# jzi040941/PercepNet

Hardware: AMD Instinct MI355X
Metric: real-time 48 kHz streams (10 ms frames), whole job (higher is better)
Workload: dtype f32; 1 GPU; configs[2]: 65536 concurrent 48 kHz streams per MI355X, fp32 network as MFMA GEMM; streams_per_gpu=65536, frame_samples=480, nn_mode=mfma_f32, weights=torch.manual_seed(1234) default-init PercepNet in nnet_data.h layout, parallelism=streams sharded over 1 GPU(s), one process per GPU, no data-path collective, io=int16 PCM in, int16 PCM + g|r rows out, resident in HBM, distributed=none (plain process)

## Files before the change

### percepnet_amd/build.py

```python
import os
import subprocess
import sys

HERE = os.path.dirname(os.path.abspath(__file__))
CSRC = os.path.join(HERE, "csrc")
LIBDIR = os.path.join(HERE, "lib")
LIB = os.path.join(LIBDIR, "libpercepnet_hip.so")
RUN = os.path.join(LIBDIR, "percepnet_run")
EXPORT_MAP = os.path.join(CSRC, "libpercepnet_hip.map")
SOURCES = ["pn_tables.cpp", "pn_model.cpp", "pn_pack.cpp", "pn_dsp_fe.hip", "pn_dsp_fe_g2.hip", "pn_dsp_fe_split_s.hip", "pn_dsp_fe_split_p.hip", "pn_dsp.hip", "pn_outstage.hip", "pn_nn.hip", "pn_nn_small.hip", "pn_nn_x3.hip", "pn_nn_d.hip", "pn_nn_n48.hip", "pn_targets.hip", "pn_state.hip", "pn_active.hip", "pn_stream_state.hip", "pn_context.cpp", "pn_selftest.cpp", "pn_host_pipe.cpp", "pn_stream_state.cpp", "pn_network.cpp",
           "pn_featgen.cpp", "pn_rate.hip", "pn_rate.cpp", "rnnoise_compat.cpp"]
FLAGS = ["--offload-arch=gfx950", "-O3", "-std=c++17", "-ffp-contract=off", "-fPIC", "-fvisibility=hidden",
         "-Wall", "-Wno-unused-function", "-Wno-unused-variable", "-Wno-unused-value", "-Wno-unused-result"]


EXTRA_FLAGS = {"pn_nn_x3.hip": ["-fno-slp-vectorize", "-mllvm", "-pragma-unroll-threshold=1000000"],
               "pn_nn_d.hip": ["-fno-slp-vectorize"]}


def _hipcc():
    for c in (os.environ.get("HIPCC"), "/opt/rocm/bin/hipcc", "hipcc"):
        if c and (os.path.isabs(c) and os.path.exists(c) or not os.path.isabs(c)):
            return c
    raise RuntimeError("hipcc not found")


EXPECTED_HIP = "7.2"

RESOURCE_LIMITS = {"pn_fe_spec_in_kernel": (0, 0), "pn_fe_spec_out_kernel": (0, 40), "pn_fe_pitch_kernel": (0, 48),
                   "pn_backend_kernel": (0, 16),
                   "pn_gru_x3_kernel": (0, 0), "pn_dense_x3_kernel": (0, 0),
                   "pn_gru_d_kernel": (0, 0)}
RESOURCE_SOURCES = ("pn_dsp_fe_split_s.hip", "pn_dsp_fe_split_p.hip", "pn_dsp.hip", "pn_nn_x3.hip", "pn_nn_d.hip")


def parse_resource_remarks(text):
    import re
    out, cur = {}, None
    for line in text.splitlines():
        m = re.search(r"remark: .*Function Name: (\S+)", line)
        if m:
            name = m.group(1)
            mm = re.match(r"_Z\d+(pn_[a-z0-9_]+)", name)
            cur = out.setdefault(name, {"kernel": mm.group(1) if mm else name})
            continue
        m = re.search(r"remark: .*?\s+(VGPRs|AGPRs|ScratchSize \[bytes/lane\]|Occupancy \[waves/SIMD\]|LDS Size \[bytes/block\]|VGPRs Spill|SGPRs Spill): (\d+)", line)
        if m and cur is not None:
            cur[m.group(1).split(" [")[0]] = int(m.group(2))
    return out


def check_resources(remarks):
    bad = []
    for name, r in remarks.items():
        for prefix, (max_agpr, max_scratch) in RESOURCE_LIMITS.items():
            if r["kernel"].startswith(prefix):
                if r.get("AGPRs", 0) > max_agpr or r.get("ScratchSize", 0) > max_scratch:
                    bad.append(f"{r['kernel']}: {r.get('VGPRs')} VGPRs, {r.get('AGPRs')} AGPRs, {r.get('ScratchSize')} B/lane scratch "
                               f"(limits: {max_agpr} AGPRs, {max_scratch} B) [{name}]")
    return bad


LLVM_BIN = "/opt/rocm/lib/llvm/bin"
GATED_OBJECTS = ("pn_dsp_fe_split_p",)


def disassemble_device_code(obj_path):
    import shutil
    import tempfile
    objdump = os.path.join(LLVM_BIN, "llvm-objdump")
    if not os.path.exists(objdump):
        objdump = shutil.which("llvm-objdump")
    if not objdump:
        raise RuntimeError("llvm-objdump not found: the disassembly gate cannot run")
    with tempfile.TemporaryDirectory() as d:
        local = os.path.join(d, os.path.basename(obj_path))
        shutil.copy(obj_path, local)
        subprocess.run([objdump, "--offloading", local], cwd=d, capture_output=True, text=True, check=True)
        cos = [f for f in os.listdir(d) if "amdgcn" in f]
        if not cos:
            raise RuntimeError(f"no device code object in {obj_path}")
        return subprocess.run([objdump, "-d", os.path.join(d, cos[0])], capture_output=True, text=True, check=True).stdout


def _vregs(op):
    import re
    m = re.fullmatch(r"v(\d+)", op)
    if m:
        return {int(m.group(1))}
    m = re.fullmatch(r"v\[(\d+):(\d+)\]", op)
    return set(range(int(m.group(1)), int(m.group(2)) + 1)) if m else set()


def check_dpp_and_waitcnt(disasm):
    import re
    bad = []
    func, ins = None, []
    funcs = {}
    for line in disasm.splitlines():
        m = re.match(r"^[0-9a-f]+ <([^>]+)>:", line)
        if m:
            func = m.group(1); ins = funcs.setdefault(func, [])
            continue
        t = line.split("//")[0].strip()
        if func is None or not t or t.startswith("."):
            continue
        parts = t.split(None, 1)
        ops = [o.strip() for o in re.split(r",\s*(?![^\[]*\])", parts[1])] if len(parts) > 1 else []
        ins.append((parts[0], ops, t))
    for func, ins in funcs.items():
        for i, (mn, ops, text) in enumerate(ins):
            if "_dpp" not in mn or len(ops) < 2:
# ... 134 lines not shown
```

### percepnet_amd/csrc/pn_context.cpp

```cpp
#include "pn_context.h"
#include <stdio.h>
#include <float.h>
#include <math.h>

extern "C" int pn_device_count(void) { int n = 0; return hipGetDeviceCount(&n) == hipSuccess ? n : 0; }


static thread_local bool g_last_alloc_oom = false;
bool &last_alloc_oom() { return g_last_alloc_oom; }
int dev_alloc_into(std::vector<void *> &allocs, size_t &total, hipStream_t stream, void **p, size_t bytes, bool zero) {
  static const bool guard = getenv("PERCEPNET_GUARD") != NULL;
  const size_t pad = guard ? (1u << 20) : 0, body = (bytes + 255) & ~(size_t)255;
  {
    const hipError_t e = hipMalloc(p, guard ? body + pad : bytes);
    if (e != hipSuccess) {
      g_last_alloc_oom = (e == hipErrorOutOfMemory);
      (void)hipGetLastError();
      pn_set_error("hipMalloc(%zu bytes) failed: %s", bytes, hipGetErrorString(e));
      return -1;
    }
  }
  allocs.push_back(*p);
  total += bytes;
  if (zero) PN_HIP_CHECK(hipMemsetAsync(*p, 0, bytes, stream));
// ... 160 lines not shown
  }
  return 0;
}
extern "C" int pn_ctx_n_streams(const pn_ctx *c) { return c ? c->B : -1; }
extern "C" int64_t pn_ctx_frames_done(const pn_ctx *c) { return c ? c->t : -1; }
extern "C" size_t pn_ctx_device_bytes(const pn_ctx *c) { return c ? c->bytes + ((c->weights && !c->weights_were_cached) ? c->weight_bytes : 0) : 0; }
extern "C" size_t pn_ctx_weight_bytes(const pn_ctx *c) { return (c && c->weights) ? c->weight_bytes : 0; }
extern "C" int pn_ctx_describe(const pn_ctx *c, char *buf, size_t n) {
  if (!c || !buf || !n) return -1;
  const int f = pn_plan_describe(c->plan, c->nn_mode, buf, n);
  if (f < 0 || (size_t)f >= n) return -1;
  const int k = c->plan.chains;
  const int w = f + snprintf(buf + f, n - f, " weights=%s nn_chains=%d%s%s", c->weights_were_cached ? "shared" : "own", k, k > 1 ? ":" : "", k > 1 ? c->chain_kind + 1 : "");
  if (w < 0 || (size_t)w >= n) return -1;
  if (c->x3_sat) {
    DeviceGuard _dg(c->device);
    hipStreamSynchronize(c->stream);
    const int w2 = snprintf(buf + w, n - w, " x3_saturated=%lld", pn_x3_sat_read());
    return (w2 < 0 || (size_t)(w + w2) >= n) ? -1 : w + w2;
  }
  return w;
}
extern "C" int pn_ctx_synchronize(pn_ctx *c) { if (!c) return -1; PN_ON_DEVICE(c); PN_HIP_CHECK(hipStreamSynchronize(c->stream)); return 0; }


static int flush_events(pn_ctx *c) {
  PN_HIP_CHECK(hipStreamSynchronize(c->stream));
  for (int k = 1; k < 4; k++) if (c->chain_stream[k]) PN_HIP_CHECK(hipStreamSynchronize(c->chain_stream[k]));
  for (auto &e : c->events) {
    float ms = 0;
    if (hipEventElapsedTime(&ms, e.a, e.b) == hipSuccess) { c->fam_ms[e.fam] += ms; c->fam_n[e.fam]++; }
    c->event_pool.push_back(e.a); c->event_pool.push_back(e.b);
  }
  c->events.clear();
  return 0;
}

extern "C" int pn_ctx_set_profiling(pn_ctx *c, int enable) {
  if (!c) return -1;
  if (enable && c->event_pool.size() < 2048) {
    PN_ON_DEVICE(c);
    while (c->event_pool.size() < 2048) { hipEvent_t e; PN_HIP_CHECK(hipEventCreate(&e)); c->event_pool.push_back(e); }
  }
  c->profiling = enable != 0;
  return 0;
}
extern "C" int pn_kernel_count(void) { return KF_COUNT; }
extern "C" const char *pn_kernel_name(int i) { return (i >= 0 && i < KF_COUNT) ? pn_kFamilyName[i] : NULL; }
extern "C" int pn_ctx_kernel_time(pn_ctx *c, const char *name, double *total_ms, int64_t *launches) {
  if (!c || !name) return -1;
  if (flush_events(c)) return -1;
  for (int i = 0; i < KF_COUNT; i++)
    if (!strcmp(name, pn_kFamilyName[i])) { if (total_ms) *total_ms = c->fam_ms[i]; if (launches) *launches = c->fam_n[i]; return 0; }
  pn_set_error("unknown kernel family '%s'", name);
  return -1;
}
extern "C" int pn_ctx_reset_profile(pn_ctx *c) {
  if (!c) return -1;
  if (flush_events(c)) return -1;
  memset(c->fam_ms, 0, sizeof(c->fam_ms)); memset(c->fam_n, 0, sizeof(c->fam_n));
  return 0;
}

void pn_launch_fe(hipStream_t st, const PnTables *T, int n_streams, int fe, int k, const PnDspSide &s, const PnDspSlots &sl, const PnDspIn &in, int grid_cap) {
  static PnFeLaunch *const launch[][3] = {{pn_launch_frontend}, {pn_launch_frontend_g2}, {pn_launch_fe_spec_in, pn_launch_fe_pitch, pn_launch_fe_spec_out}};
  static_assert(sizeof(launch) / sizeof(launch[0]) == sizeof(pn_kFe) / sizeof(pn_kFe[0]) && sizeof(launch[0]) / sizeof(launch[0][0]) == sizeof(pn_kFe[0].fam) / sizeof(int),
                "one row of launchers per front-end family of pn_kFe");
  launch[fe][k](st, T, n_streams, s, sl, in, grid_cap);
}

int process_dev(pn_ctx *c, const void *d_in, void *d_out, float *d_gr, int is_i16) {
  if (!c || !d_in || !d_out) { pn_set_error("NULL argument"); return -1; }
  PN_ON_DEVICE(c);
  const PnDspSide &s = c->side;
  const PnDspSlots k = pn_dsp_slots(c->t);
  const PnDspIn in = {d_in, is_i16, PN_FRAME, 1.f / 32768.f};
  float *const gr = c->st[PN_ST_GR].p;
  for (int i = 0; i < pn_kFe[c->plan.fe].n; i++) {
    Scope sc(c, pn_kFe[c->plan.fe].fam[i]);
    pn_launch_fe(c->stream, c->tables, c->B, c->plan.fe, i, s, k, in, c->dsp_grid_cap);
  }
  if (launch_rnn(c)) return -1;
  const bool stage = c->report_on || (c->saturate && is_i16), staged_cast = stage && is_i16;
  { Scope sc(c, KF_BACKEND);
    pn_launch_backend(c->stream, c->tables, c->B, pn_dsp_spec(s, k.slot_r), s.Ps, gr, c->postfilter ? pn_dsp_bands(s, k.slot_r) : nullptr, s.silence,
                      c->st[PN_ST_SYNTH].p, staged_cast ? (void *)c->stage_o : d_out, staged_cast ? 0 : is_i16, c->dsp_grid_cap,
                      c->n_limited > 0 ? c->lam_mu : nullptr); }
  if (stage) {
    Scope sc(c, KF_BACKEND);
    pn_launch_outstage(c->stream, c->B, staged_cast ? c->stage_o : (const float *)d_out, s, (k.frame_t + 6) % PN_HIST_FRAMES, gr,
                       is_i16 ? (int16_t *)d_out : nullptr, c->saturate, c->report_on ? c->report : nullptr);
  }
  if (d_gr) PN_HIP_CHECK(hipMemcpyAsync(d_gr, gr, (size_t)c->B * 68 * 4, hipMemcpyDeviceToDevice, c->stream));
  PN_HIP_CHECK(hipGetLastError());
  c->t++; c->tn++;
  if (c->events.size() >= 4096 && flush_events(c)) return -1;
  return 0;
}

extern "C" int pn_ctx_debug_inject_launch_failure(pn_ctx *c, int enable) {
  if (!c) { pn_set_error("NULL argument"); return -1; }
  c->inject_bad_launch = enable != 0;
  return 0;
}

extern "C" int pn_ctx_set_postfilter(pn_ctx *c, int enable) {
  if (!c) { pn_set_error("NULL argument"); return -1; }
  c->postfilter = enable != 0;
  return 0;
}

static int stage_buffers(pn_ctx *c, bool report) {
  if (!c->stage_o && dev_alloc(c, (void **)&c->stage_o, (size_t)c->B * PN_FRAME * sizeof(float), false)) return -1;
  if (report && !c->report && dev_alloc(c, (void **)&c->report, (size_t)c->B * PN_REPORT_WORDS * 4, true)) return -1;
  return 0;
}
extern "C" int pn_ctx_set_report(pn_ctx *c, int enable) {
  if (!c) { pn_set_error("NULL argument"); return -1; }
  if (enable) { PN_ON_DEVICE(c); if (stage_buffers(c, true)) return -1; }
  else c->next_report = NULL;
  c->report_on = enable != 0;
  return 0;
}
extern "C" int pn_ctx_set_output_saturate(pn_ctx *c, int enable) {
  if (!c) { pn_set_error("NULL argument"); return -1; }
  if (enable) { PN_ON_DEVICE(c); if (stage_buffers(c, false)) return -1; }
  c->saturate = enable != 0;
  return 0;
}
static int report_copy(pn_ctx *c, void *dst, hipMemcpyKind kind) {
  if (!c || !dst) { pn_set_error("NULL argument"); return -1; }
  if (!c->report_on) { pn_set_error("the frame report is off (pn_ctx_set_report)"); return -1; }
  PN_ON_DEVICE(c);
  PN_HIP_CHECK(hipMemcpyAsync(dst, c->report, (size_t)c->B * PN_REPORT_WORDS * 4, kind, c->stream));
  if (kind == hipMemcpyDeviceToHost) PN_HIP_CHECK(hipStreamSynchronize(c->stream));
  return 0;
}
extern "C" int pn_ctx_read_report(pn_ctx *c, void *h_report) { return report_copy(c, h_report, hipMemcpyDeviceToHost); }
extern "C" int pn_ctx_read_report_dev(pn_ctx *c, void *d_report) { return report_copy(c, d_report, hipMemcpyDeviceToDevice); }

extern "C" float pn_atten_limit_factor(float db) {
  if (!(db >= 0.f)) return NAN;
  const float lam = (float)pow(10.0, -(double)db / 20.0);
  return lam < FLT_MIN ? 0.f : lam;
}
extern "C" int pn_ctx_set_atten_limit(pn_ctx *c, const int32_t *ids, int n, const float *db) {
  if (!c || (n > 0 && !db)) { pn_set_error("bad argument"); return -1; }
  if (pn_ids_check(c->B, ids, n, true)) return -1;
  if (n == 0) return 0;
  for (int i = 0; i < n; i++) {
    if (!(db[i] >= 0.f)) { pn_set_error("attenuation limit %g dB for stream %d: must be >= 0 (+inf = off)", (double)db[i], ids[i]); return -1; }
  }
  PN_ON_DEVICE(c);
  if (!c->lam_mu && dev_alloc(c, (void **)&c->lam_mu, (size_t)c->B * sizeof(float2), true)) return -1;
  std::vector<float2> lm(n);
  for (int i = 0; i < n; i++) { const float lam = pn_atten_limit_factor(db[i]); lm[i] = make_float2(lam, 1.0f - lam); }
  const int *d = stage_ids(c, ids, n, lm.data(), 2 * n);
  if (!d) return -1;
  pn_launch_scatter_pairs(c->stream, c->lam_mu, d, reinterpret_cast<const float2 *>(d + stage_payload_offset(n)), n);
  PN_HIP_CHECK(hipGetLastError());
  for (int i = 0; i < n; i++) {
    c->n_limited += (lm[i].x != 0.f) - (pn_atten_limit_factor(c->atten_db[ids[i]]) != 0.f);
    c->atten_db[ids[i]] = db[i];
  }
  return 0;
}
extern "C" int pn_ctx_get_atten_limit(const pn_ctx *c, float *h_db) {
  if (!c || !h_db) { pn_set_error("bad argument"); return -1; }
  memcpy(h_db, c->atten_db.data(), (size_t)c->B * sizeof(float));
  return 0;
}

extern "C" int pn_process_f32(pn_ctx *c, const float *d_in, float *d_out, float *d_gr) { return process_dev(c, d_in, d_out, d_gr, 0); }
extern "C" int pn_process_i16(pn_ctx *c, const int16_t *d_in, int16_t *d_out, float *d_gr) { return process_dev(c, d_in, d_out, d_gr, 1); }
extern "C" int pn_process_i16_multi(pn_ctx *c, const int16_t *d_in, int16_t *d_out, float *d_gr, int n_frames) {
  if (!c) return -1;
// ... 106 lines not shown
```

### percepnet_amd/csrc/pn_dsp.hip

```cpp
#include "pn_fft960.h"
#include "pn_launch.h"
#include "pn_pcm.h"

#define LANES 64
#ifndef PN_DSP_WPB
#define PN_DSP_WPB 8
#endif
#ifndef PN_DSP_WAVES_PER_SIMD
#define PN_DSP_WAVES_PER_SIMD 4
#endif
#define WPB PN_DSP_WPB
#define DSP_THREADS (LANES * WPB)

#define PN_WAVE_SYNC_GLOBAL() do { __builtin_amdgcn_fence(__ATOMIC_SEQ_CST, "workgroup"); __builtin_amdgcn_wave_barrier(); } while (0)

struct alignas(16) PnDspWaveLds {
  float2 fft[FS_NF];
  float e[4][PN_NB + 2];
};
struct PnDspShared {
  float win[PN_FRAME];
  float frac[PN_SPEC_BINS];
  uint8_t band[PN_SPEC_BINS];
  PnDspWaveLds w[WPB];
};

template <typename P, typename... R> __device__ __forceinline__ P pn_first_arg(P p, R...) { return p; }

template <typename TOut, bool PF, typename... LamMu>
__global__ __launch_bounds__(DSP_THREADS, PN_DSP_WAVES_PER_SIMD) void pn_backend_kernel(
    const PnTables *__restrict__ T, int n_streams,
    const float2 *__restrict__ Xspec, const float2 *__restrict__ Pspec,
    const float *__restrict__ gr,
    const float *__restrict__ ex,
    const int *__restrict__ silence,
    float *__restrict__ synth_mem,
    TOut *__restrict__ out,
    const LamMu *__restrict__... lam_mu) {
  constexpr bool AL = sizeof...(LamMu) != 0;
  __shared__ PnDspShared SH;
  const int tid = threadIdx.x, lane = tid & (LANES - 1), wave = __builtin_amdgcn_readfirstlane(tid >> 6);
  for (int i = tid; i < PN_FRAME; i += DSP_THREADS) SH.win[i] = T->half_window[i];
  for (int i = tid; i < PN_SPEC_BINS; i += DSP_THREADS) { SH.frac[i] = T->bin_frac[i]; SH.band[i] = T->bin_band[i]; }
  __syncthreads();
  PnDspWaveLds &W = SH.w[wave];
  FsLane Z;
  fs_lane_init(Z, T, lane);
  const float scale = 1.f / PN_NFFT;
  const int lc = lane < 60 ? lane : 59;
  for (int s = blockIdx.x * WPB + wave; s < n_streams; s += gridDim.x * WPB) {
    const bool sil = silence[s] != 0;
    float lam = 0.f, mu = 0.f;
    if constexpr (AL) { const float2 lm = pn_first_arg(lam_mu...)[s]; lam = lm.x; mu = lm.y; }
    const bool mix = AL && lam != 0.f;
    if (lane < PN_NB) {
      const float g = gr[(size_t)s * 68 + lane], r = gr[(size_t)s * 68 + PN_NB + lane];
      W.e[0][lane] = g; W.e[1][lane] = r; W.e[2][lane] = 1 - r;
      if (PF) W.e[3][lane] = ex[(size_t)s * 36 + lane];
    }
    PN_WAVE_SYNC();
    if (PF) {
      float gw = 0.f;
      float *gws = reinterpret_cast<float *>(W.fft);
      if (lane < PN_NB) { const float g = W.e[0][lane]; gw = g * sinf((float)(M_PI / 2 * (double)g)); gws[lane] = gw; }
      PN_WAVE_SYNC();
      float E0 = 0.f, E1 = 0.f;
#pragma unroll 2
      for (int i = 0; i < PN_NB; i++) {
        const float e = W.e[3][i];
        E0 += W.e[0][i] * e;
        E1 += gws[i] * e;
      }
      const float E_div = E0 / (E1 + 1e-6f);
      const float G = sqrtf(((1 + 0.02f) * E_div) / (1 + 0.02f * (E_div * E_div)));
      PN_WAVE_SYNC();
      if (lane < PN_NB) W.e[0][lane] = G * gw;
      PN_WAVE_SYNC();
    }
    {
      const float4 *X4 = reinterpret_cast<const float4 *>(Xspec + (size_t)s * PN_SPEC_BINS);
      const float4 *P4 = reinterpret_cast<const float4 *>(Pspec + (size_t)s * PN_SPEC_BINS);
      float4 xq[4], pq[4];
      int la = lane;
      asm volatile("" : "+v"(la));
#pragma unroll
      for (int it = 0; it < 4; it++) {
        const int m = la + 64 * it, mc = m < PN_SPEC_BINS / 2 ? m : PN_SPEC_BINS / 2 - 1;
        xq[it] = X4[mc];
        pq[it] = sil ? make_float4(0.f, 0.f, 0.f, 0.f) : P4[mc];
      }
      float4 *Y4 = reinterpret_cast<float4 *>(W.fft);
#pragma unroll
      for (int it = 0; it < 4; it++) {
        const int m = la + 64 * it;
        if (m < PN_SPEC_BINS / 2) {
          float2 y[2];
#pragma unroll
          for (int h = 0; h < 2; h++) {
            const int k = 2 * m + h;
            float2 x = h ? make_float2(xq[it].z, xq[it].w) : make_float2(xq[it].x, xq[it].y);
            const int b = SH.band[k];
            const float fr = SH.frac[k];
            if (!sil) {
              const float2 p = h ? make_float2(pq[it].z, pq[it].w) : make_float2(pq[it].x, pq[it].y);
              const float rf1 = (1 - fr) * W.e[2][b] + fr * W.e[2][b + 1];
              x.x = rf1 * x.x; x.y = rf1 * x.y;
              const float rf2 = (1 - fr) * W.e[1][b] + fr * W.e[1][b + 1];
              x.x += rf2 * p.x; x.y += rf2 * p.y;
            }
            const float gf = (1 - fr) * W.e[0][b] + fr * W.e[0][b + 1];
            x.x *= gf; x.y *= gf;
            if constexpr (AL)
              if (mix) {
                const float2 a = h ? make_float2(xq[it].z, xq[it].w) : make_float2(xq[it].x, xq[it].y);
                x.x = (mu * x.x) + (lam * a.x); x.y = (mu * x.y) + (lam * a.y);
              }
            y[h] = make_float2(scale * x.x, scale * x.y);
          }
          Y4[m] = make_float4(y[0].x, y[0].y, y[1].x, y[1].y);
        }
      }
    }
    PN_WAVE_SYNC();
    __builtin_amdgcn_sched_barrier(0);
    {
      float2 fin[4][4];
      int lq = lc;
      asm volatile("" : "+v"(lq));
      const float2 *Yd = W.fft + 4 * lq, *Ym = W.fft + (PN_WINDOW - 4 * lq);
#pragma unroll
      for (int c = 0; c < 4; c++)
#pragma unroll
        for (int j = 0; j < 4; j++) {
          const int o = c + 240 * j, kk = j < 2 ? 4 * lq + o : PN_WINDOW - 4 * lq - o;
          float2 x = j < 2 ? Yd[o] : Ym[-o];
          if (kk >= PN_SPEC_BINS) x = make_float2(0.f, 0.f);
          if (j == 3 || (j == 2 && (c > 0 || lq > 0))) x.y = -x.y;
          fin[c][j] = x;
        }
      PN_WAVE_SYNC();
      if (lane < 60) {
#pragma unroll
        for (int c = 0; c < 4; c++) {
          fs_bfly4_m1(fin[c]);
          float4 *dst = reinterpret_cast<float4 *>(W.fft + Z.p1off[c]);
          dst[0] = make_float4(fin[c][0].x, fin[c][0].y, fin[c][1].x, fin[c][1].y);
          dst[1] = make_float4(fin[c][2].x, fin[c][2].y, fin[c][3].x, fin[c][3].y);
        }
      }
    }
    __builtin_amdgcn_sched_barrier(0);
    float2 w[3][5];
    fs_fft_p23<true>(W.fft, T, lane, w);
    float *sm = synth_mem + (size_t)s * PN_FRAME;
    float smv[15];
#pragma unroll
    for (int q = 0; q < 15; q++) {
      const int p = lane + 64 * (q % 3) + 192 * (q / 3);
      const bool lo = p == 0 || p > PN_FRAME;
      smv[q] = lo ? sm[p == 0 ? 0 : PN_WINDOW - p] : 0.f;
    }
    PN_WAVE_SYNC_GLOBAL();
#pragma unroll
    for (int q = 0; q < 15; q++) {
      const int p = lane + 64 * (q % 3) + 192 * (q / 3);
      const float re = w[q % 3][q / 3].x;
      if (p == 0 || p > PN_FRAME) {
        const int i = p == 0 ? 0 : PN_WINDOW - p;
        const float o = (PN_WINDOW * re) * SH.win[i] + smv[q];
        if (sizeof(TOut) == 2) out[(size_t)s * PN_FRAME + i] = (TOut)pn_f2s(o * 32768);
        else out[(size_t)s * PN_FRAME + i] = (TOut)o;
      } else {
        sm[PN_FRAME - p] = (PN_WINDOW * re) * SH.win[p - 1];
      }
    }
    PN_WAVE_SYNC();
  }
}

static inline int pn_dsp_grid(int n_streams, int blocks_per_cu, int grid_cap) {
  const int need = (n_streams + WPB - 1) / WPB;
  const int full = PN_DSP_WAVES_PER_SIMD * 4 / WPB;
  const int cap = grid_cap > 0 ? grid_cap : 256 * ((blocks_per_cu > 0 && blocks_per_cu < full) ? blocks_per_cu : full);
  return need < cap ? need : cap;
}

template <typename TOut, bool PF, typename... LamMu>
static void backend_launch(hipStream_t st, int grid, const PnTables *T, int n_streams, const float2 *Xs, const float2 *Ps, const float *gr,
                           const float *ex, const int *silence, float *synth_mem, void *out, const float2 *lam_mu) {
  if constexpr (sizeof...(LamMu) != 0)
    hipLaunchKernelGGL((pn_backend_kernel<TOut, PF, LamMu...>), dim3(grid), dim3(DSP_THREADS), 0, st, T, n_streams, Xs, Ps, gr, ex, silence, synth_mem,
                       (TOut *)out, lam_mu);
  else
    hipLaunchKernelGGL((pn_backend_kernel<TOut, PF>), dim3(grid), dim3(DSP_THREADS), 0, st, T, n_streams, Xs, Ps, gr, ex, silence, synth_mem, (TOut *)out);
}
void pn_launch_backend(hipStream_t st, const PnTables *T, int n_streams, const float2 *Xs, const float2 *Ps,
                       const float *gr, const float *ex_postfilter, const int *silence, float *synth_mem, void *out,
                       int out_is_i16, int grid_cap, const float2 *lam_mu) {
  static constexpr decltype(&backend_launch<float, false>) launch[2][2][2] = {
      {{backend_launch<int16_t, true, float2>, backend_launch<float, true, float2>},
       {backend_launch<int16_t, false, float2>, backend_launch<float, false, float2>}},
      {{backend_launch<int16_t, true>, backend_launch<float, true>},
       {backend_launch<int16_t, false>, backend_launch<float, false>}}};
  const int limited_off = !lam_mu, pf_off = !ex_postfilter, i16_off = !out_is_i16;
  launch[limited_off][pf_off][i16_off](st, pn_dsp_grid(n_streams, 0, grid_cap), T, n_streams, Xs, Ps, gr, ex_postfilter, silence, synth_mem, out, lam_mu);
}
```

### percepnet_amd/csrc/pn_dsp_fe_split_s.hip

```cpp
#define PN_FE_G 1
#include "pn_dsp_fe_helpers.inc"

#define FS_WPB 4
#define FS_THREADS (LANES * FS_WPB)
#include "pn_fft960.h"
#include "pn_launch.h"
#include <stdlib.h>

#ifndef PN_FS_WAVES_IN
#define PN_FS_WAVES_IN 4
#endif
#ifndef PN_FS_PREFETCH
#define PN_FS_PREFETCH 1
#endif
#ifndef PN_FS_WAVES_OUT
#define PN_FS_WAVES_OUT 3
#endif
struct FsShared {
  float2 f[FS_WPB][FS_NF];
  float win[PN_FRAME];
  float frac[PN_SPEC_BINS];
  unsigned pos[PN_SPEC_BINS];
};

#define FS_NBIN 7
struct FsBands {
  const float *frac;
  const unsigned *pos;
  int start, nq;
};
__device__ __forceinline__ void fs_bands_init(FsBands &B, const FsShared &SH, const PnTables *__restrict__ T, int l) {
  B.frac = SH.frac; B.pos = SH.pos;
  B.start = l < PN_NB ? T->band_start[l] : 0;
  B.nq = l < PN_NB ? T->band_nq[l] : 0;
}
__device__ __forceinline__ void fs_bands_fill(float *C, const FsBands &B, const float *tmp, int l) {
#pragma unroll
  for (int it = 0; it < (PN_BAND_LAYOUT_FLOATS / 4 + 63) / 64; it++) {
    const int q = l + 64 * it;
    if (q < PN_BAND_LAYOUT_FLOATS / 4) *reinterpret_cast<float4 *>(C + 4 * q) = make_float4(0.f, 0.f, 0.f, 0.f);
  }
  float fr[FS_NBIN]; unsigned ps[FS_NBIN];
#pragma unroll
  for (int j = 0; j < FS_NBIN; j++) {
    const int k = (j < 6) ? l + 64 * j : (l < 16 ? 384 + l : 0);
    fr[j] = B.frac[k]; ps[j] = B.pos[k];
  }
#pragma unroll
  for (int j = 0; j < FS_NBIN; j++) {
    if (j == 6 && l >= 16) continue;
    const float fa = fr[j] * tmp[j], fb = (1 - fr[j]) * tmp[j];
    C[ps[j] & 0xffff] = fa;
    C[ps[j] >> 16] = fb;
  }
}
template <int NARR>
__device__ __forceinline__ void fs_bands_sum(const float *C, const FsBands &B, int l, float *sum) {
#pragma unroll
  for (int h = 0; h < NARR; h++) sum[h] = 0;
  const float *p = C + B.start;
  for (int q = 0; q < 25; q++) {
    if (q < B.nq) {
#pragma unroll
      for (int h = 0; h < NARR; h++) {
        const float4 v = *reinterpret_cast<const float4 *>(p + h * PN_BAND_LAYOUT_FLOATS + 4 * q);
        sum[h] += v.x; sum[h] += v.y; sum[h] += v.z; sum[h] += v.w;
      }
    }
  }
  if (l == 0 || l == PN_NB - 1)
#pragma unroll
    for (int h = 0; h < NARR; h++) sum[h] *= 2;
}

template <typename TIn>
__global__ __launch_bounds__(FS_THREADS, PN_FS_WAVES_IN) void pn_fe_spec_in_kernel(
    const PnTables *__restrict__ T, int n_streams, int frame_t, int slot_w,
    const TIn *__restrict__ in, long long in_stride, float i16_scale,
    float *__restrict__ hist, float2 *__restrict__ yring, float *__restrict__ eyring) {
  __shared__ FsShared SH;
  const int tid = threadIdx.x, l = tid & (LANES - 1), wave = __builtin_amdgcn_readfirstlane(tid >> 6);
  float2 *F = SH.f[wave];
  float *C = reinterpret_cast<float *>(F);
  for (int i = tid; i < PN_FRAME; i += FS_THREADS) SH.win[i] = T->half_window[i];
  for (int i = tid; i < PN_SPEC_BINS; i += FS_THREADS) {
    SH.frac[i] = T->bin_frac[i];
    SH.pos[i] = (unsigned)T->band_pos_a[i] | ((unsigned)T->band_pos_b[i] << 16);
  }
  __syncthreads();
  FsLane Z; FsBands B;
  fs_lane_init(Z, T, l);
  fs_bands_init(B, SH, T, l);
  const int new_slot = frame_t % PN_HIST_FRAMES;
  const int prev_slot = (frame_t + PN_HIST_FRAMES - 1) % PN_HIST_FRAMES;
  const int lc = l < 60 ? l : 59;
  for (int s = blockIdx.x * FS_WPB + wave; s < n_streams; s += gridDim.x * FS_WPB) {
// ... 41 lines not shown
  }
}

__device__ __forceinline__ void fs_spec_out_tail(const float4 *x, const float2 *__restrict__ Xr, float Ex, float Ey, int s, int l, float2 *F, float *C,
                                                 const FsShared &SH, const FsLane &Z, const FsBands &B, const PnTables *__restrict__ T,
                                                 float2 *__restrict__ Pspec, float *__restrict__ feat, int *__restrict__ silence, float *__restrict__ aux) {
  fs_fft_p1(F, SH.win, Z, x, l);
  float2 w[3][5];
  fs_fft_p23<false>(F, T, l, w);
  const float2 o2 = w[0][2];
  float2 xv[FS_NBIN];
#pragma unroll
  for (int j = 0; j < FS_NBIN; j++) xv[j] = Xr[(j < 6) ? l + 64 * j : (l < 16 ? 384 + l : 0)];
  float tp[FS_NBIN], tx[FS_NBIN];
#pragma unroll
  for (int j = 0; j < FS_NBIN; j++) {
    const float2 P = j < 6 ? w[j % 3][j / 3] : o2;
    if (j < 6 || l < 16) Pspec[(size_t)s * PN_SPEC_BINS + (j < 6 ? l + 64 * j : 384 + l)] = P;
    float t = P.x * P.x; t += P.y * P.y; tp[j] = t;
    float u = xv[j].x * P.x; u += xv[j].y * P.y; tx[j] = u;
  }
  PN_WAVE_SYNC();
  fs_bands_fill(C, B, tp, l);
  fs_bands_fill(C + PN_BAND_LAYOUT_FLOATS, B, tx, l);
  PN_WAVE_SYNC();
  float sums[2];
  fs_bands_sum<2>(C, B, l, sums);
  const float Ep = sums[0];
  float Exp = sums[1];
  float *f = feat + (size_t)s * PN_FEAT_STRIDE;
  if (l < PN_NB) {
    Exp = (float)fmin(1.0, fmax(0.0, (double)Exp / sqrt(1e-15 + (double)(Ex * Ep))));
    f[l] = Ey * 30;
    f[PN_NB + l] = Exp * 30;
    if (aux) { aux[(size_t)s * PN_AUX_STRIDE + l] = Ep; aux[(size_t)s * PN_AUX_STRIDE + PN_NB + l] = Exp; }
  }
  {
    float E = 0;
#pragma unroll
    for (int i = 0; i < PN_NB; i++) E += __shfl(Ex, i);
    if (l == 0) silence[s] = ((double)E < 0.1) ? 1 : 0;
  }
  PN_WAVE_SYNC();
}

__global__ __launch_bounds__(FS_THREADS, PN_FS_WAVES_OUT) void pn_fe_spec_out_kernel(
    const PnTables *__restrict__ T, int n_streams, int frame_t, int slot_w, int slot_r,
    const float *__restrict__ hist, const float2 *__restrict__ yring, const float *__restrict__ eyring,
    const int *__restrict__ last_period,
    float2 *__restrict__ Pspec, float *__restrict__ feat, int *__restrict__ silence, float *__restrict__ aux) {
  __shared__ FsShared SH;
  const int tid = threadIdx.x, l = tid & (LANES - 1), wave = __builtin_amdgcn_readfirstlane(tid >> 6);
  float2 *F = SH.f[wave];
  float *C = reinterpret_cast<float *>(F);
  for (int i = tid; i < PN_FRAME; i += FS_THREADS) SH.win[i] = T->half_window[i];
  for (int i = tid; i < PN_SPEC_BINS; i += FS_THREADS) {
    SH.frac[i] = T->bin_frac[i];
    SH.pos[i] = (unsigned)T->band_pos_a[i] | ((unsigned)T->band_pos_b[i] << 16);
  }
  __syncthreads();
  FsLane Z; FsBands B;
  fs_lane_init(Z, T, l);
  fs_bands_init(B, SH, T, l);
  float cw[7];
#pragma unroll
  for (int k = 0; k < 7; k++) cw[k] = T->comb_hann[k];
  const int base_slot0 = (frame_t + 1) % PN_HIST_FRAMES;
  const int lc = l < 60 ? l : 59;
#if PN_FS_PREFETCH & 1
  int period_next = 0;
  { const int s0 = blockIdx.x * FS_WPB + wave; if (s0 < n_streams) period_next = last_period[s0]; }
#endif
  for (int s = blockIdx.x * FS_WPB + wave; s < n_streams; s += gridDim.x * FS_WPB) {
    const float *h = hist + (size_t)s * PN_HIST_STRIDE;
#if PN_FS_PREFETCH & 1
    const int pitch_index = period_next;
    { const int sn = s + gridDim.x * FS_WPB; period_next = last_period[sn < n_streams ? sn : s]; }
#else
    const int pitch_index = last_period[s];
#endif
    int base_slot = base_slot0;
    asm volatile("" : "+v"(base_slot));
    const float2 *Xr = yring + ((size_t)slot_r * n_streams + s) * PN_SPEC_BINS;
    const float Ex = l < PN_NB ? eyring[((size_t)slot_r * n_streams + s) * 36 + l] : 0.f;
    const float Ey = l < PN_NB ? eyring[((size_t)slot_w * n_streams + s) * 36 + l] : 0.f;
    float4 x[4];
    int bs = base_slot;
#pragma unroll
    for (int k0 = 0; k0 < 4; k0 += 2) {
      if (k0) asm volatile("" : "+v"(bs) : "v"(x[1].w));
      fe_f4u cv[2][7];
#pragma unroll
      for (int q = 0; q < 2; q++)
#pragma unroll
        for (int k = -PN_COMB_M; k <= PN_COMB_M; k++)
          cv[q][k + PN_COMB_M] = *reinterpret_cast<const fe_f4u *>(h + fe_ring(2400 - pitch_index * k + 4 * lc + 240 * (k0 + q), bs));
#pragma unroll
      for (int q = 0; q < 2; q++) {
        float p[4];
#pragma unroll
        for (int c = 0; c < 4; c++) {
          float acc = 0;
#pragma unroll
          for (int k = 0; k < 7; k++) acc += cv[q][k][c] * cw[k];
          p[c] = acc;
        }
        x[k0 + q] = make_float4(p[0], p[1], p[2], p[3]);
      }
    }
    fs_spec_out_tail(x, Xr, Ex, Ey, s, l, F, C, SH, Z, B, T, Pspec, feat, silence, aux);
  }
}


static int fs_grid(int n_streams, int blocks_per_cu, int grid_cap) {
  const int need = (n_streams + FS_WPB - 1) / FS_WPB;
  const int cap = grid_cap > 0 ? grid_cap : 256 * blocks_per_cu;
  return need < cap ? need : cap;
}
void pn_launch_fe_spec_in(hipStream_t st, const PnTables *T, int n_streams, const PnDspSide &s, const PnDspSlots &k, const PnDspIn &in, int grid_cap) {
  if (in.is_i16)
    hipLaunchKernelGGL(pn_fe_spec_in_kernel<int16_t>, dim3(fs_grid(n_streams, PN_FS_WAVES_IN, grid_cap)), dim3(FS_THREADS), 0, st, T, n_streams, k.frame_t,
                       k.slot_w, (const int16_t *)in.p, in.stride, in.i16_scale, s.hist, s.yring, s.eyring);
  else
    hipLaunchKernelGGL(pn_fe_spec_in_kernel<float>, dim3(fs_grid(n_streams, PN_FS_WAVES_IN, grid_cap)), dim3(FS_THREADS), 0, st, T, n_streams, k.frame_t,
                       k.slot_w, (const float *)in.p, in.stride, in.i16_scale, s.hist, s.yring, s.eyring);
}
void pn_launch_fe_spec_out(hipStream_t st, const PnTables *T, int n_streams, const PnDspSide &s, const PnDspSlots &k, const PnDspIn &, int grid_cap) {
  hipLaunchKernelGGL(pn_fe_spec_out_kernel, dim3(fs_grid(n_streams, PN_FS_WAVES_OUT, grid_cap)), dim3(FS_THREADS), 0, st, T, n_streams, k.frame_t, k.slot_w,
                     k.slot_r, s.hist, s.yring, s.eyring, s.last_period, s.Ps, s.feat, s.silence, s.aux);
}
```

### percepnet_amd/csrc/pn_featgen.cpp

```cpp
#include "pn_context.h"
#include <stdlib.h>
#include <string.h>
#include <vector>

struct pn_featgen {
  int device, B; int64_t t; size_t bytes;
  int fe;
  hipStream_t stream; bool own_stream;
  PnTables *tables;
  float *st[2][PN_ST_COUNT];
  PnDspSide clean, noisy;
  float *synth;
  float *gr, *tmp_out;
  std::vector<void *> allocs;
};

static int fg_alloc(pn_featgen *c, float **p, size_t words) { return dev_alloc_into(c->allocs, c->bytes, c->stream, (void **)p, words * 4, true); }

extern "C" void pn_featgen_destroy(pn_featgen *c) {
  if (!c) return;
  DeviceGuard _dg(c->device);
  hipStreamSynchronize(c->stream);
  for (void *p : c->allocs) hipFree(p);
  if (c->own_stream) hipStreamDestroy(c->stream);
  delete c;
}

extern "C" pn_featgen *pn_featgen_create(int device, int n_pairs, void *hip_stream) {
  if (n_pairs < 1) { pn_set_error("n_pairs must be >= 1"); return NULL; }
  DeviceGuard _dg; hipStream_t stream; bool own_stream;
  if (open_device(device, hip_stream, _dg, &stream, &own_stream)) return NULL;
  pn_featgen *c = new pn_featgen();
  c->device = device; c->B = n_pairs; c->t = 0; c->bytes = 0; c->fe = pn_plan_for(n_pairs, PN_NN_MFMA).fe;
  c->stream = stream; c->own_stream = own_stream;
  const size_t B = n_pairs;
  if (tables_upload(c->allocs, c->bytes, c->stream, &c->tables, NULL)) goto fail;
  for (int side = 0; side < 2; side++) {
    float *aux;
    for (int e : pn_kSideEntries)
      if (fg_alloc(c, &c->st[side][e], pn_state_size(pn_kState[e], B).words)) goto fail;
    if (fg_alloc(c, &aux, B * PN_AUX_STRIDE)) goto fail;
    (side ? c->noisy : c->clean) = pn_dsp_side(c->st[side], aux, B);
  }
  if (fg_alloc(c, &c->synth, pn_state_size(pn_kState[PN_ST_SYNTH], B).words) || fg_alloc(c, &c->gr, pn_state_size(pn_kState[PN_ST_GR], B).words) ||
      fg_alloc(c, &c->tmp_out, B * PN_FRAME)) goto fail;
  if (hipStreamSynchronize(c->stream) != hipSuccess) { pn_set_error("featgen init failed"); goto fail; }
  return c;
fail:
  pn_featgen_destroy(c);
  return NULL;
}

extern "C" int pn_featgen_reset(pn_featgen *c) {
  if (!c) return -1;
  PN_ON_DEVICE(c);
  for (int side = 0; side < 2; side++)
    for (int e : pn_kSideEntries) PN_HIP_CHECK(hipMemsetAsync(c->st[side][e], 0, pn_state_size(pn_kState[e], c->B).words * 4, c->stream));
  PN_HIP_CHECK(hipMemsetAsync(c->synth, 0, pn_state_size(pn_kState[PN_ST_SYNTH], c->B).words * 4, c->stream));
  c->t = 0;
  return 0;
}
extern "C" int pn_featgen_n_pairs(const pn_featgen *c) { return c ? c->B : -1; }
extern "C" int64_t pn_featgen_frames_done(const pn_featgen *c) { return c ? c->t : -1; }
extern "C" size_t pn_featgen_device_bytes(const pn_featgen *c) { return c ? c->bytes : 0; }
extern "C" int pn_featgen_synchronize(pn_featgen *c) { if (!c) return -1; PN_HIP_CHECK(hipStreamSynchronize(c->stream)); return 0; }

static int fg_frame(pn_featgen *c, const int16_t *sp, const int16_t *no, long long in_stride, float *rec,
                    long long rec_stride, int16_t *pcm, long long pcm_stride) {
  const PnDspSlots k = pn_dsp_slots(c->t);
  const PnDspSide *side[2] = {&c->noisy, &c->clean};
  const PnDspIn in[2] = {{no, 1, in_stride, 1.f}, {sp, 1, in_stride, 1.f}};
  for (int s = 0; s < 2; s++)
    for (int i = 0; i < pn_kFe[c->fe].n; i++) pn_launch_fe(c->stream, c->tables, c->B, c->fe, i, *side[s], k, in[s], 0);
  pn_launch_targets(c->stream, c->tables, c->B, pn_dsp_bands(c->clean, k.slot_r), pn_dsp_bands(c->noisy, k.slot_r), pn_dsp_bands(c->noisy, k.slot_w),
                    c->clean.aux, c->noisy.aux, c->noisy.last_period, rec, rec_stride, c->gr);
  pn_launch_backend(c->stream, c->tables, c->B, pn_dsp_spec(c->noisy, k.slot_r), c->noisy.Ps, c->gr,
                    nullptr , c->noisy.silence, c->synth, c->tmp_out, 0, 0,
                    nullptr );
  if (pcm) pn_launch_saturate_i16(c->stream, c->B, c->tmp_out, pcm, pcm_stride);
  PN_HIP_CHECK(hipGetLastError());
  c->t++;
  return 0;
}

extern "C" int pn_featgen_process_i16(pn_featgen *c, const int16_t *d_speech, const int16_t *d_noisy, float *d_records,
                                      int16_t *d_test_pcm) {
  if (!c || !d_speech || !d_noisy || !d_records) { pn_set_error("NULL argument"); return -1; }
  PN_ON_DEVICE(c);
  return fg_frame(c, d_speech, d_noisy, PN_FRAME, d_records, 138, d_test_pcm, PN_FRAME);
}

extern "C" int pn_featgen_process_i16_files(pn_featgen *c, const int16_t *d_speech, const int16_t *d_noisy,
                                            int n_frames, float *d_records, int16_t *d_test_pcm) {
  if (!c || !d_speech || !d_noisy || !d_records || n_frames < 0) { pn_set_error("bad argument"); return -1; }
  PN_ON_DEVICE(c);
  const long long in_stride = (long long)n_frames * PN_FRAME;
  for (int f = 0; f < n_frames; f++)
    if (fg_frame(c, d_speech + (size_t)f * PN_FRAME, d_noisy + (size_t)f * PN_FRAME, in_stride,
                 d_records + (size_t)f * 138, (long long)n_frames * 138,
                 d_test_pcm ? d_test_pcm + (size_t)f * PN_FRAME : NULL, in_stride))
      return -1;
  return 0;
}

extern "C" int pn_featgen_process_host_i16_files(pn_featgen *c, const int16_t *h_speech, const int16_t *h_noisy,
                                                 int n_frames, float *h_records, int16_t *h_test_pcm) {
  if (!c || !h_speech || !h_noisy || !h_records || n_frames < 0) { pn_set_error("bad argument"); return -1; }
  PN_ON_DEVICE(c);
  const size_t n_in = (size_t)c->B * n_frames * PN_FRAME, n_rec = (size_t)c->B * n_frames * 138;
  int16_t *d_sp = NULL, *d_no = NULL, *d_pcm = NULL; float *d_rec = NULL;
  int rc = -1;
  do {
    if (hipMalloc((void **)&d_sp, n_in * 2) != hipSuccess || hipMalloc((void **)&d_no, n_in * 2) != hipSuccess ||
        hipMalloc((void **)&d_rec, n_rec * 4) != hipSuccess ||
        (h_test_pcm && hipMalloc((void **)&d_pcm, n_in * 2) != hipSuccess)) { pn_set_error("hipMalloc failed (featgen staging)"); break; }
    if (hipMemcpyAsync(d_sp, h_speech, n_in * 2, hipMemcpyHostToDevice, c->stream) != hipSuccess ||
        hipMemcpyAsync(d_no, h_noisy, n_in * 2, hipMemcpyHostToDevice, c->stream) != hipSuccess) { pn_set_error("H2D failed"); break; }
    if (pn_featgen_process_i16_files(c, d_sp, d_no, n_frames, d_rec, d_pcm)) break;
    if (hipMemcpyAsync(h_records, d_rec, n_rec * 4, hipMemcpyDeviceToHost, c->stream) != hipSuccess ||
        (h_test_pcm && hipMemcpyAsync(h_test_pcm, d_pcm, n_in * 2, hipMemcpyDeviceToHost, c->stream) != hipSuccess)) { pn_set_error("D2H failed"); break; }
    if (hipStreamSynchronize(c->stream) != hipSuccess) { pn_set_error("stream sync failed: %s", hipGetErrorString(hipGetLastError())); break; }
    rc = 0;
  } while (0);
  hipStreamSynchronize(c->stream);
  hipFree(d_sp); hipFree(d_no); hipFree(d_rec); hipFree(d_pcm);
  return rc;
}

static bool fg_read_pcm(const char *path, std::vector<int16_t> &v) {
  FILE *f = fopen(path, "rb");
  if (!f) return false;
  fseek(f, 0, SEEK_END); long n = ftell(f); fseek(f, 0, SEEK_SET);
  v.resize(n > 0 ? (size_t)n / 2 : 0);
  const size_t got = v.empty() ? 0 : fread(v.data(), 2, v.size(), f);
  fclose(f);
  v.resize(got / PN_FRAME * PN_FRAME);
  return true;
}

extern "C" int pn_featgen_run_files(int device, int n_jobs, const char *const *speech_paths,
                                    const char *const *noisy_paths, const int *counts, const char *const *out_paths,
                                    const char *const *test_out_paths, const char *const *test_in_paths) {
  if (n_jobs < 1 || !speech_paths || !noisy_paths || !counts || !out_paths) { pn_set_error("bad argument"); return -1; }
  std::vector<std::vector<int16_t>> sp(n_jobs), no(n_jobs);
  std::vector<FILE *> fo(n_jobs, NULL), fto(n_jobs, NULL), fti(n_jobs, NULL);
  int rc = -1, max_count = 0;
  pn_featgen *fg = NULL;
  auto close_all = [&]() {
    for (int j = 0; j < n_jobs; j++) { if (fo[j]) fclose(fo[j]); if (fto[j]) fclose(fto[j]); if (fti[j]) fclose(fti[j]); }
  };
  for (int j = 0; j < n_jobs; j++) {
    if (!fg_read_pcm(speech_paths[j], sp[j]) || !fg_read_pcm(noisy_paths[j], no[j])) {
      pn_set_error("cannot read %s / %s", speech_paths[j], noisy_paths[j]); close_all(); return -1; }
    if (counts[j] > 0 && (sp[j].size() < PN_FRAME || no[j].size() < PN_FRAME)) {
      pn_set_error("job %d: inputs must hold at least one 480-sample frame", j); close_all(); return -1; }
    fo[j] = fopen(out_paths[j], "wb");
    if (!fo[j]) { pn_set_error("cannot create %s", out_paths[j]); close_all(); return -1; }
    if (test_out_paths && test_out_paths[j]) fto[j] = fopen(test_out_paths[j], "wb");
    if (test_in_paths && test_in_paths[j]) fti[j] = fopen(test_in_paths[j], "wb");
    if (counts[j] > max_count) max_count = counts[j];
  }
// ... 38 lines not shown
```

### percepnet_amd/csrc/pn_launch.h

```cpp
#pragma once
#include "pn_common.h"
#include "pn_network.h"

typedef void PnFeLaunch(hipStream_t st, const PnTables *T, int n_streams, const PnDspSide &s, const PnDspSlots &k, const PnDspIn &in, int grid_cap);
PnFeLaunch pn_launch_frontend;
PnFeLaunch pn_launch_frontend_g2;
PnFeLaunch pn_launch_fe_spec_in, pn_launch_fe_pitch, pn_launch_fe_spec_out;
void pn_launch_fe(hipStream_t st, const PnTables *T, int n_streams, int fe, int k, const PnDspSide &s, const PnDspSlots &sl, const PnDspIn &in, int grid_cap);
void pn_launch_zero_rows(hipStream_t st, void *base, int row_floats, long long row_stride, int n_slots, long long slot_stride,
                         const int *d_ids, int n);
void pn_launch_zero_shadow_rows(hipStream_t st, void *S, int width, int np, int n_slots, long long slot_stride_halfs,
                                const int *d_ids, int n);
void pn_launch_scatter_pairs(hipStream_t st, float2 *dst, const int *d_ids, const float2 *d_vals, int n);
struct PnSsSection { float *base; uint4 *shadow; long long row_stride, slot_stride; int slots, first, live, cols, rec_off, np; };
struct PnActiveArgs {
  const int *ids;
  float *synth; int *last_period; float *last_gain;
  void *out; int out_row_words; float *d_gr;
  float *save_synth; uint32_t *save_out; float *save_gr; int *save_period; float *save_gain;
  PnSsSection sec[PN_SS_NSEC];
  int restore_only;
};
void pn_launch_inactive_save(hipStream_t st, const PnActiveArgs &a, int n);
int pn_launch_spin(hipStream_t st, long long ticks);
void pn_launch_inactive_fixup(hipStream_t st, const PnActiveArgs &a, int n);
struct PnStreamStateArgs {
  PnSsSection sec[PN_SS_NSEC];
  float *last_gain; int *last_period;
  const int *ids;
  void *rec;
  int *status;
  uint32_t hdr[16];
};
void pn_launch_ss_gather(hipStream_t st, const PnStreamStateArgs &a, int n);
void pn_launch_ss_scatter(hipStream_t st, const PnStreamStateArgs &a, int n);
int pn_launch_split_x3_rows(hipStream_t st, const float *src, int ld, int width, void *S, const int *d_ids, const int *d_status, int n, int np);
int pn_launch_split_d_rows(hipStream_t st, const float *src, int ld, int width, void *S, const int *d_ids, const int *d_status, int n);
void pn_launch_targets(hipStream_t st, const PnTables *T, int n_pairs, const float *ex_clean, const float *ex_noisy,
                       const float *ey_look_noisy, const float *aux_clean, const float *aux_noisy,
                       const int *period_noisy, float *records, long long rec_stride, float *gr);
void pn_launch_saturate_i16(hipStream_t st, int n_pairs, const float *in, int16_t *out, long long out_stride);
void pn_launch_backend(hipStream_t st, const PnTables *T, int n_streams, const float2 *Xs, const float2 *Ps,
                       const float *gr, const float *ex_postfilter , const int *silence, float *synth_mem,
                       void *out, int out_is_i16, int grid_cap,
                       const float2 *lam_mu );
void pn_launch_outstage(hipStream_t st, int n_streams, const float *o, const PnDspSide &s, int hist_slot, const float *gr,
                        int16_t *pcm, int saturate, void *report);
int pn_launch_rate_up(hipStream_t st, int factor, int is_i16, int n_rows, const int *d_ids, const void *in, float *out48, float *tail, const float *taps);
int pn_launch_rate_down(hipStream_t st, int factor, int is_i16, int n_rows, const int *d_ids, const float *in48, void *out, int saturate, float *tail, const float *taps);
void pn_launch_rate_records(hipStream_t st, int factor, int rate_hz, const int *d_ids, int n, float *tail_up, float *tail_down, int td_stride, void *rec, int scatter);
int pn_launch_rate_up_mixed(hipStream_t st, int is_i16, int n_rows, const int *d_ids, const int *d_factors, const void *in, float *out48, float *tail, const float *taps);
int pn_launch_rate_down_mixed(hipStream_t st, int is_i16, int n_rows, const int *d_ids, const int *d_factors, const float *in48, void *out, int saturate, float *tail, const float *taps);
void pn_launch_rate_records_dev(hipStream_t st, const int *d_ids, int n, const int *d_factors, int factor, float *tail_up, float *tail_down, int td_stride,
                                void *rec, int stride_words, int *d_status, int scatter);
void pn_launch_rate_set_factors(hipStream_t st, const int *d_ids, const int *d_vals, int n, int *d_factors);
struct DevLayer { float *bias, *w, *rw, *wp, *rwp, *wq; };
struct PnLayerLaunch {
  PnSegs A, S;
  const float *bias;
  const void *w, *rw;
  int N, act; const float *tansig;
  float *out; int ldo;
  void *outS; int nts_out;
  const float *h_old; const void *h_oldS;
  int n_rows, rg, np;
};
typedef int PnLayerLauncher(hipStream_t, const PnLayerLaunch &);
PnLayerLauncher pn_launch_dense_strict, pn_launch_gru_strict, pn_launch_dense, pn_launch_gru;
PnLayerLauncher pn_launch_dense_small, pn_launch_gru_small, pn_launch_dense_n16, pn_launch_dense_n48;
PnLayerLauncher pn_launch_dense_x3, pn_launch_gru_x3, pn_launch_gru_d;
size_t pn_packed_halfs_x3(int k_alloc, int ncols, int ct_round, int np );
int pn_pack_weights_x3(const float *W, int K, int k_alloc, int ncols, int ct_round, int np, void *Wp);
int pn_x3_sat_set(int enable);
long long pn_x3_sat_read();
int pn_launch_split_x3(hipStream_t st, const float *src, int ld, int width, void *S, int n_rows_padded, int np);
int pn_launch_split_d(hipStream_t st, const float *src, int ld, int width, void *S, int n_rows);
```

Before: 72400 streams.

## Write g|r rows from backend kernel and defer Ex/Ey loads in spec_out

Measured after the change: 72480 streams (median of 6 runs). About the same (+0.1%).

```diff
diff --git a/percepnet_amd/build.py b/percepnet_amd/build.py
--- a/percepnet_amd/build.py
+++ b/percepnet_amd/build.py
@@ -27,7 +27,7 @@
 
 EXPECTED_HIP = "7.2"
 
-RESOURCE_LIMITS = {"pn_fe_spec_in_kernel": (0, 0), "pn_fe_spec_out_kernel": (0, 40), "pn_fe_pitch_kernel": (0, 48),
+RESOURCE_LIMITS = {"pn_fe_spec_in_kernel": (0, 0), "pn_fe_spec_out_kernel": (0, 0), "pn_fe_pitch_kernel": (0, 48),
                    "pn_backend_kernel": (0, 16),
                    "pn_gru_x3_kernel": (0, 0), "pn_dense_x3_kernel": (0, 0),
                    "pn_gru_d_kernel": (0, 0)}
diff --git a/percepnet_amd/csrc/pn_context.cpp b/percepnet_amd/csrc/pn_context.cpp
--- a/percepnet_amd/csrc/pn_context.cpp
+++ b/percepnet_amd/csrc/pn_context.cpp
@@ -266,16 +266,17 @@
   }
   if (launch_rnn(c)) return -1;
   const bool stage = c->report_on || (c->saturate && is_i16), staged_cast = stage && is_i16;
+  float *const gr_direct = PN_BE_GR_DIRECT ? d_gr : nullptr;
   { Scope sc(c, KF_BACKEND);
     pn_launch_backend(c->stream, c->tables, c->B, pn_dsp_spec(s, k.slot_r), s.Ps, gr, c->postfilter ? pn_dsp_bands(s, k.slot_r) : nullptr, s.silence,
                       c->st[PN_ST_SYNTH].p, staged_cast ? (void *)c->stage_o : d_out, staged_cast ? 0 : is_i16, c->dsp_grid_cap,
-                      c->n_limited > 0 ? c->lam_mu : nullptr); }
+                      c->n_limited > 0 ? c->lam_mu : nullptr, gr_direct); }
   if (stage) {
     Scope sc(c, KF_BACKEND);
     pn_launch_outstage(c->stream, c->B, staged_cast ? c->stage_o : (const float *)d_out, s, (k.frame_t + 6) % PN_HIST_FRAMES, gr,
                        is_i16 ? (int16_t *)d_out : nullptr, c->saturate, c->report_on ? c->report : nullptr);
   }
-  if (d_gr) PN_HIP_CHECK(hipMemcpyAsync(d_gr, gr, (size_t)c->B * 68 * 4, hipMemcpyDeviceToDevice, c->stream));
+  if (d_gr && !gr_direct) PN_HIP_CHECK(hipMemcpyAsync(d_gr, gr, (size_t)c->B * 68 * 4, hipMemcpyDeviceToDevice, c->stream));
   PN_HIP_CHECK(hipGetLastError());
   c->t++; c->tn++;
   if (c->events.size() >= 4096 && flush_events(c)) return -1;
diff --git a/percepnet_amd/csrc/pn_dsp.hip b/percepnet_amd/csrc/pn_dsp.hip
--- a/percepnet_amd/csrc/pn_dsp.hip
+++ b/percepnet_amd/csrc/pn_dsp.hip
@@ -36,6 +36,7 @@
     const int *__restrict__ silence,
     float *__restrict__ synth_mem,
     TOut *__restrict__ out,
+    float *__restrict__ gr_out,
     const LamMu *__restrict__... lam_mu) {
   constexpr bool AL = sizeof...(LamMu) != 0;
   __shared__ PnDspShared SH;
@@ -56,6 +57,7 @@
     if (lane < PN_NB) {
       const float g = gr[(size_t)s * 68 + lane], r = gr[(size_t)s * 68 + PN_NB + lane];
       W.e[0][lane] = g; W.e[1][lane] = r; W.e[2][lane] = 1 - r;
+      if (gr_out) { gr_out[(size_t)s * 68 + lane] = g; gr_out[(size_t)s * 68 + PN_NB + lane] = r; }
       if (PF) W.e[3][lane] = ex[(size_t)s * 36 + lane];
     }
     PN_WAVE_SYNC();
@@ -187,21 +189,21 @@
 
 template <typename TOut, bool PF, typename... LamMu>
 static void backend_launch(hipStream_t st, int grid, const PnTables *T, int n_streams, const float2 *Xs, const float2 *Ps, const float *gr,
-                           const float *ex, const int *silence, float *synth_mem, void *out, const float2 *lam_mu) {
+                           const float *ex, const int *silence, float *synth_mem, void *out, float *gr_out, const float2 *lam_mu) {
   if constexpr (sizeof...(LamMu) != 0)
     hipLaunchKernelGGL((pn_backend_kernel<TOut, PF, LamMu...>), dim3(grid), dim3(DSP_THREADS), 0, st, T, n_streams, Xs, Ps, gr, ex, silence, synth_mem,
-                       (TOut *)out, lam_mu);
+                       (TOut *)out, gr_out, lam_mu);
   else
-    hipLaunchKernelGGL((pn_backend_kernel<TOut, PF>), dim3(grid), dim3(DSP_THREADS), 0, st, T, n_streams, Xs, Ps, gr, ex, silence, synth_mem, (TOut *)out);
+    hipLaunchKernelGGL((pn_backend_kernel<TOut, PF>), dim3(grid), dim3(DSP_THREADS), 0, st, T, n_streams, Xs, Ps, gr, ex, silence, synth_mem, (TOut *)out, gr_out);
 }
 void pn_launch_backend(hipStream_t st, const PnTables *T, int n_streams, const float2 *Xs, const float2 *Ps,
                        const float *gr, const float *ex_postfilter, const int *silence, float *synth_mem, void *out,
-                       int out_is_i16, int grid_cap, const float2 *lam_mu) {
+                       int out_is_i16, int grid_cap, const float2 *lam_mu, float *gr_out) {
   static constexpr decltype(&backend_launch<float, false>) launch[2][2][2] = {
       {{backend_launch<int16_t, true, float2>, backend_launch<float, true, float2>},
        {backend_launch<int16_t, false, float2>, backend_launch<float, false, float2>}},
       {{backend_launch<int16_t, true>, backend_launch<float, true>},
        {backend_launch<int16_t, false>, backend_launch<float, false>}}};
   const int limited_off = !lam_mu, pf_off = !ex_postfilter, i16_off = !out_is_i16;
-  launch[limited_off][pf_off][i16_off](st, pn_dsp_grid(n_streams, 0, grid_cap), T, n_streams, Xs, Ps, gr, ex_postfilter, silence, synth_mem, out, lam_mu);
-}
+  launch[limited_off][pf_off][i16_off](st, pn_dsp_grid(n_streams, 0, grid_cap), T, n_streams, Xs, Ps, gr, ex_postfilter, silence, synth_mem, out, gr_out, lam_mu);
+}
diff --git a/percepnet_amd/csrc/pn_dsp_fe_split_s.hip b/percepnet_amd/csrc/pn_dsp_fe_split_s.hip
--- a/percepnet_amd/csrc/pn_dsp_fe_split_s.hip
+++ b/percepnet_amd/csrc/pn_dsp_fe_split_s.hip
@@ -12,6 +12,9 @@
 #endif
 #ifndef PN_FS_PREFETCH
 #define PN_FS_PREFETCH 1
+#endif
+#ifndef PN_FS_E_AFTER_COMB
+#define PN_FS_E_AFTER_COMB 1
 #endif
 #ifndef PN_FS_WAVES_OUT
 #define PN_FS_WAVES_OUT 3
@@ -219,8 +222,12 @@
     int base_slot = base_slot0;
     asm volatile("" : "+v"(base_slot));
     const float2 *Xr = yring + ((size_t)slot_r * n_streams + s) * PN_SPEC_BINS;
-    const float Ex = l < PN_NB ? eyring[((size_t)slot_r * n_streams + s) * 36 + l] : 0.f;
+#define FS_LOAD_EXY()                                                                                                         \
+    const float Ex = l < PN_NB ? eyring[((size_t)slot_r * n_streams + s) * 36 + l] : 0.f;                        \
     const float Ey = l < PN_NB ? eyring[((size_t)slot_w * n_streams + s) * 36 + l] : 0.f;
+#if !PN_FS_E_AFTER_COMB
+    FS_LOAD_EXY()
+#endif
     float4 x[4];
     int bs = base_slot;
 #pragma unroll
@@ -245,6 +252,10 @@
         x[k0 + q] = make_float4(p[0], p[1], p[2], p[3]);
       }
     }
+#if PN_FS_E_AFTER_COMB
+    FS_LOAD_EXY()
+#endif
+#undef FS_LOAD_EXY
     fs_spec_out_tail(x, Xr, Ex, Ey, s, l, F, C, SH, Z, B, T, Pspec, feat, silence, aux);
   }
 }
diff --git a/percepnet_amd/csrc/pn_featgen.cpp b/percepnet_amd/csrc/pn_featgen.cpp
--- a/percepnet_amd/csrc/pn_featgen.cpp
+++ b/percepnet_amd/csrc/pn_featgen.cpp
@@ -76,7 +76,7 @@
                     c->clean.aux, c->noisy.aux, c->noisy.last_period, rec, rec_stride, c->gr);
   pn_launch_backend(c->stream, c->tables, c->B, pn_dsp_spec(c->noisy, k.slot_r), c->noisy.Ps, c->gr,
                     nullptr , c->noisy.silence, c->synth, c->tmp_out, 0, 0,
-                    nullptr );
+                    nullptr , nullptr );
   if (pcm) pn_launch_saturate_i16(c->stream, c->B, c->tmp_out, pcm, pcm_stride);
   PN_HIP_CHECK(hipGetLastError());
   c->t++;
diff --git a/percepnet_amd/csrc/pn_launch.h b/percepnet_amd/csrc/pn_launch.h
--- a/percepnet_amd/csrc/pn_launch.h
+++ b/percepnet_amd/csrc/pn_launch.h
@@ -40,10 +40,14 @@
                        const float *ey_look_noisy, const float *aux_clean, const float *aux_noisy,
                        const int *period_noisy, float *records, long long rec_stride, float *gr);
 void pn_launch_saturate_i16(hipStream_t st, int n_pairs, const float *in, int16_t *out, long long out_stride);
+#ifndef PN_BE_GR_DIRECT
+#define PN_BE_GR_DIRECT 1
+#endif
 void pn_launch_backend(hipStream_t st, const PnTables *T, int n_streams, const float2 *Xs, const float2 *Ps,
                        const float *gr, const float *ex_postfilter , const int *silence, float *synth_mem,
                        void *out, int out_is_i16, int grid_cap,
-                       const float2 *lam_mu );
+                       const float2 *lam_mu ,
+                       float *gr_out);
 void pn_launch_outstage(hipStream_t st, int n_streams, const float *o, const PnDspSide &s, int hist_slot, const float *gr,
                         int16_t *pcm, int saturate, void *report);
 int pn_launch_rate_up(hipStream_t st, int factor, int is_i16, int n_rows, const int *d_ids, const void *in, float *out48, float *tail, const float *taps);
```
